# psc0628/NeRF-PRV

Hardware: AMD Instinct MI355X
Metric: ray-samples/s (field evaluations composited; candidate views rendered + scored; scene baseline, field 256^3) (higher is better)
Workload: dtype f16

## Files before the change

### nerf_prv_amd/csrc/prv_api.cpp

```cpp
#include <hip/hip_runtime.h>

#include <algorithm>
#include <atomic>
#include <chrono>
#include <cmath>
#include <cstdarg>
#include <cstdio>
#include <cstdlib>
#include <cstring>
#include <memory>
#include <new>
#include <stdexcept>
#include <string>
#include <vector>

#include "prv_json.hpp"
#include "prv_kernels.hpp"
#include "prv_mesh.hpp"
#include "prv_levels.hpp"
#include "prv_ingp.hpp"
#include "prv_train.hpp"

using namespace prv;

// ... 29 lines not shown
  CamDev* dev = nullptr;
  int device = 0;
  int width = 0, height = 0;
  bool dataset = false;
};

static void train_detach_all(struct prv_ctx* c);
static void comm_detach_all(struct prv_ctx* c);
static void mesh_detach_all(struct prv_ctx* c);

struct prv_ctx {
  int device = 0;
  int n_cu = 256;
  hipStream_t own_stream = nullptr;
  hipStream_t stream = nullptr;
  std::vector<hipStream_t> idle_queues;
  hipStream_t capture_stream = nullptr;
  std::vector<Buffer> idle_buffers;
  size_t idle_bytes = 0;
  std::string err;
  Model models[PRV_MAX_SLOTS];
  Buffer queue, queue_ext, stage, counters, view_ids, img_f32, partial, records, dbg[6];
  Buffer stage_depth;
  Buffer counters_multi, occ_multi;
  int march_multi = -1;
  Buffer img_u8[PRV_MAX_MODELS];
  bool profiling = false;
  std::vector<hipEvent_t> ev_render, ev_march;
  std::vector<hipEvent_t> ev_free;
  std::vector<float> last_render_ms;
  void* pin = nullptr;
  size_t pin_cap = 0;
  hipEvent_t pin_ev = nullptr;
  int blocks_per_cu = -1;
  int cell_cache = -1;
  std::vector<struct prv_trainer*> trainers;
  std::vector<struct prv_comm*> comms;
  std::vector<struct prv_mesh*> meshes;
  float mesh_ms[4] = {0, 0, 0, 0};
  int queue_segments = 8;
  int spatial_regions = 1;
  int pool_on = -1;
  int merge_max = -1;
  size_t stage_budget = (size_t)4 << 30;
  size_t queue_budget = (size_t)8 << 30;
  double coverage_weight = PRV_COVERAGE_WEIGHT_DEFAULT;
// ... 490 lines not shown
  }
  if (!c->pin_ev) HIPCHK(c, hipEventCreateWithFlags(&c->pin_ev, hipEventDisableTiming));
  else HIPCHK(c, hipEventSynchronize(c->pin_ev));
  CamDev* cams = (CamDev*)c->pin;
  int* ids = (int*)((char*)c->pin + (size_t)n_views * sizeof(CamDev));
  int rc;
  if ((rc = gather_cams(c, cs, view_ids, n_views, W, H, cams)) != PRV_OK) return rc;
  for (int i = 0; i < n_views; i++) {
    set_cull_rect(cams[i], box, W, H);
    ids[i] = i;
  }
  if ((rc = ensure(c, c->view_ids, up_bytes)) != PRV_OK) return rc;
  HIPCHK(c, hipMemcpyAsync(c->view_ids.p, c->pin, up_bytes, hipMemcpyHostToDevice, c->stream));
  HIPCHK(c, hipEventRecord(c->pin_ev, c->stream));
  up.cams = cams;
  up.cams_dev = (const CamDev*)c->view_ids.p;
  up.ids_dev = (const int*)((char*)c->view_ids.p + (size_t)n_views * sizeof(CamDev));
  return PRV_OK;
}

constexpr int kSubRegions = 8, kMaxSegments = 8 * kSubRegions;
constexpr size_t kStatOffset = (size_t)kMaxSegments * 128;
constexpr size_t kCountersBytes = kStatOffset + 72 * 8;

struct MarchLayout {
  int spp, n_sub, n_seg;
  int spp_inner_log2 = 0, tile_w_log2, tile_h_log2;
  uint32_t tiles_x, tiles_y;
  MarchLayout(const prv_ctx* c, int W, int H, int spp_) : spp(spp_) {
    n_sub = c->spatial_regions ? kSubRegions : 1;
    n_seg = c->queue_segments * n_sub;
    if (spp > 1 && spp <= 64 && (spp & (spp - 1)) == 0)
      while ((1 << spp_inner_log2) < spp) spp_inner_log2++;
    const int pix_log2 = 8 - spp_inner_log2;
    tile_w_log2 = (pix_log2 + 1) / 2;
    tile_h_log2 = pix_log2 / 2;
    tiles_x = (uint32_t)((W + (1 << tile_w_log2) - 1) >> tile_w_log2);
    tiles_y = (uint32_t)((H + (1 << tile_h_log2) - 1) >> tile_h_log2);
  }
  size_t blocks(size_t n_views) const { return (size_t)tiles_x * tiles_y * n_views * (size_t)(spp_inner_log2 > 0 ? 1 : spp); }
  size_t seg_cap(size_t n_views) const { return ((blocks(n_views) + n_seg - 1) / n_seg) * 256 + 64; }
};

template <class PT>
void march_common(PT& mp, const prv_ctx* c, const MarchLayout& L, const prv_render_opts* o, const Upload& up, size_t v0,
                  size_t n_views, unsigned long long* stat) {
// ... 59 lines not shown
  rp.queue_count = q.queue_count;
  rp.queue_head = queue_head;
  rp.n_segments = L.n_seg;
  rp.n_sub = L.n_sub;
  rp.seg_cap = seg_cap;
  rp.stat_evaluated = stat;
  rp.out_f32 = q.out_f32;
  rp.out_u8 = q.out_u8;
  rp.min_T = o->min_transmittance;
  rp.last_pass = o->spp == 1;
  memcpy(rp.bg, o->background, sizeof(rp.bg));
  render_policy(c, m, (size_t)o->width * o->height, o->step_mode == PRV_STEP_NGP, rp);
  return rp;
}

int render_views(prv_ctx* c, int slot, const prv_camset* cs, const int* view_ids, int n_views,
                 const prv_render_opts* o, float* out_f32, uint8_t* out_u8, bool zero_stats, bool private_output = false,
                 float* out_depth = nullptr, float* out_entropy = nullptr, float* out_alpha = nullptr) {
  if (o->spp != 1 || out_u8 || out_depth) private_output = false;
  const Model& m = c->models[slot];
  const int W = o->width, H = o->height, spp = o->spp;
  const size_t npix = (size_t)W * H;
  int rc;
  if ((rc = ensure(c, c->counters, kCountersBytes)) != PRV_OK) return rc;
  uint32_t* q_head = (uint32_t*)c->counters.p;
  uint32_t* q_count = (uint32_t*)c->counters.p + kMaxSegments * 16;
  unsigned long long* stat = (unsigned long long*)((char*)c->counters.p + kStatOffset);
  if (n_views == 0) {
    if (zero_stats) HIPCHK(c, hipMemsetAsync(stat, 0, kCountersBytes - kStatOffset, c->stream));
    return PRV_OK;
  }
  Upload up;
  if ((rc = upload_views(c, cs, view_ids, n_views, W, H, box_of(m), up)) != PRV_OK) return rc;

  const bool ngp = o->step_mode == PRV_STEP_NGP;
  const size_t slot_bytes = kRecordBytes + (ngp ? kExtBytes : 0);
  size_t batch = std::max<size_t>(1, c->queue_budget / (npix * slot_bytes * (size_t)spp));
  batch = std::min<size_t>(batch, (size_t)n_views);
  const size_t stage_px = out_entropy ? 4 + 4 : out_depth ? 16 + 4 : 16;
  if (spp > 1) batch = std::min<size_t>(batch, std::max<size_t>(1, c->stage_budget / (npix * stage_px * (size_t)spp)));
  if (batch * npix * (size_t)spp >= (1ull << 32)) batch = ((1ull << 32) - 1) / (npix * (size_t)spp);
  if (batch == 0) return fail(c, PRV_E_INVALID, "image x spp too large");
  const MarchLayout L(c, W, H, spp);
  const size_t seg_cap_max = L.seg_cap(batch);
  if (seg_cap_max * (size_t)L.n_seg >= (1ull << 32)) return fail(c, PRV_E_INVALID, "image x spp too large");
  if ((rc = ensure(c, c->queue, seg_cap_max * (size_t)L.n_seg * kRecordBytes)) != PRV_OK) return rc;
  if (ngp && (rc = ensure(c, c->queue_ext, seg_cap_max * (size_t)L.n_seg * kExtBytes)) != PRV_OK) return rc;
  if (spp > 1 && (rc = ensure(c, c->stage, batch * npix * (size_t)spp * (out_entropy ? 4 : 16))) != PRV_OK) return rc;
  if (spp > 1 && (out_depth || out_entropy) && (rc = ensure(c, c->stage_depth, batch * npix * (size_t)spp * 4)) != PRV_OK) return rc;

  const int n_blocks = render_blocks(c, m, npix);
  for (size_t b0 = 0; b0 < (size_t)n_views; b0 += batch) {
    const int nb = (int)std::min(batch, (size_t)n_views - b0);
    float* dst_f32 = out_f32 ? out_f32 + b0 * npix * 4 : nullptr;
    uint32_t* dst_u8 = out_u8 ? (uint32_t*)out_u8 + b0 * npix : nullptr;
    float* dst_depth = out_depth ? out_depth + b0 * npix : nullptr;
    float* depth_target = spp > 1 ? (float*)c->stage_depth.p : dst_depth;
    if (out_depth) HIPCHK(c, hipMemsetAsync(depth_target, 0, (size_t)nb * npix * (size_t)spp * 4, c->stream));
    float* dst_entropy = out_entropy ? out_entropy + b0 * npix : nullptr;
    float* dst_alpha = out_entropy ? out_alpha + b0 * npix : nullptr;
    float* entropy_target = spp > 1 ? (float*)c->stage_depth.p : dst_entropy;
    float* alpha_target = spp > 1 ? (float*)c->stage.p : dst_alpha;
    if (out_entropy) {
      HIPCHK(c, hipMemsetAsync(entropy_target, 0, (size_t)nb * npix * (size_t)spp * 4, c->stream));
      HIPCHK(c, hipMemsetAsync(alpha_target, 0, (size_t)nb * npix * (size_t)spp * 4, c->stream));
    }
    HIPCHK(c, hipMemsetAsync(c->counters.p, 0, b0 == 0 && zero_stats ? kCountersBytes : kStatOffset, c->stream));
    MarchParams mp;
    march_common(mp, c, L, o, up, b0, (size_t)nb, stat);
    mp.field = m.dev;
    mp.S = o->samples_per_ray;
    mp.step_mode = o->step_mode;
    mp.queue = c->queue.p;
    mp.queue_ext = (uint4*)c->queue_ext.p;
    mp.queue_count = q_count;
    mp.out_f32 = out_entropy ? nullptr : spp > 1 ? (float*)c->stage.p : dst_f32;
    mp.out_u8 = spp > 1 ? nullptr : dst_u8;
    if (private_output) {
      const uint64_t tw = 1ull << mp.tile_w_log2, th = 1ull << mp.tile_h_log2;
      uint64_t live_max = 0;
      for (int i = 0; i < nb; i++) {
        const CamDev& cv = up.cams[b0 + i];
        uint64_t w = mp.tiles_x, h = mp.tiles_y;
        if (cv.cull[2] > 0) {
          const uint64_t x0 = (uint64_t)cv.cull[0] / tw, y0 = (uint64_t)cv.cull[1] / th;
          const uint64_t x1 = std::min<uint64_t>(mp.tiles_x, ((uint64_t)cv.cull[2] + tw - 1) / tw);
          const uint64_t y1 = std::min<uint64_t>(mp.tiles_y, ((uint64_t)std::max(cv.cull[3], 0) + th - 1) / th);
          w = x1 > x0 ? x1 - x0 : 0;
          h = y1 > y0 ? y1 - y0 : 0;
        }
// ... 40 lines not shown
int render_ensemble_ngp(prv_ctx* c, const int* slots, int E, const prv_camset* cs, const int* view_ids, int n_views,
                        const prv_render_opts* o, float* scratch_f32, uint8_t* const* out_u8, bool* done) {
  *done = false;
  if (o->step_mode != PRV_STEP_NGP || !march_multi_supported(E) || n_views == 0) return PRV_OK;
  if (c->march_multi == 0) return PRV_OK;
  if (c->march_multi < 0 && E < 3) return PRV_OK;
  const Model& m0 = c->models[slots[0]];
  for (int e = 1; e < E; e++) {
    const Model& m = c->models[slots[e]];
    if (m.desc.occ_res != m0.desc.occ_res || (m.dev.occ_coarse == nullptr) != (m0.dev.occ_coarse == nullptr)) return PRV_OK;
    for (int f = 0; f < e; f++)
      if (slots[f] == slots[e]) return PRV_OK;
  }
  const int W = o->width, H = o->height, spp = o->spp;
  const size_t npix = (size_t)W * H;
  const size_t slot_bytes = kRecordBytes + kExtBytes;
  if ((size_t)n_views * npix * (size_t)spp >= (1ull << 32)) return PRV_OK;
  if ((size_t)n_views * npix * (size_t)spp * slot_bytes > c->queue_budget) return PRV_OK;
  if (spp > 1 && (size_t)n_views * npix * (size_t)spp * 16 > c->stage_budget) return PRV_OK;
  const MarchLayout L(c, W, H, spp);
  const size_t seg_cap = L.seg_cap((size_t)n_views);
  if (seg_cap * (size_t)L.n_seg >= (1ull << 32)) return PRV_OK;
  int rc;
  if ((rc = ensure(c, c->counters, kCountersBytes)) != PRV_OK) return rc;
  if ((rc = ensure(c, c->counters_multi, (size_t)E * kStatOffset)) != PRV_OK) return rc;
  unsigned long long* stat = (unsigned long long*)((char*)c->counters.p + kStatOffset);
  const size_t R = (size_t)m0.desc.occ_res, n_fine = R * R * R, Rc = R / 4, n_coarse = Rc * Rc * Rc;
  if ((rc = ensure(c, c->occ_multi, n_fine + n_coarse + 64)) != PRV_OK) return rc;
  const size_t q_stride = seg_cap * (size_t)L.n_seg * kRecordBytes, x_stride = seg_cap * (size_t)L.n_seg * kExtBytes,
               s_stride = spp > 1 ? (size_t)n_views * npix * (size_t)spp * 16 : 0;
  {
    const size_t grow = (q_stride * (size_t)E > c->queue.bytes ? q_stride * (size_t)E - c->queue.bytes : 0) +
                        (x_stride * (size_t)E > c->queue_ext.bytes ? x_stride * (size_t)E - c->queue_ext.bytes : 0) +
                        (s_stride * (size_t)E > c->stage.bytes ? s_stride * (size_t)E - c->stage.bytes : 0);
    size_t free_b = 0, total_b = 0;
    if (grow && (hipMemGetInfo(&free_b, &total_b) != hipSuccess || grow + ((size_t)2 << 30) > free_b + c->idle_bytes)) return PRV_OK;
  }

  const OccBox box = union_box(c, slots, E);
  Upload up;
  if ((rc = upload_views(c, cs, view_ids, n_views, W, H, box, up)) != PRV_OK) return rc;

  const bool have_coarse = m0.dev.occ_coarse != nullptr;
  {
    OccInterleaveParams ip{};
    ip.n_members = E;
    for (int e = 0; e < E; e++) ip.bits[e] = c->models[slots[e]].dev.occ;
    ip.n_cells = (uint32_t)n_fine;
    ip.out = (uint8_t*)c->occ_multi.p;
    HIPCHK(c, launch_occ_interleave(ip, c->stream));
    if (have_coarse) {
      for (int e = 0; e < E; e++) ip.bits[e] = c->models[slots[e]].dev.occ_coarse;
      ip.n_cells = (uint32_t)n_coarse;
      ip.out = (uint8_t*)c->occ_multi.p + n_fine;
      HIPCHK(c, launch_occ_interleave(ip, c->stream));
    }
  }

  if ((rc = ensure(c, c->queue, q_stride * (size_t)E)) != PRV_OK) return rc;
  if ((rc = ensure(c, c->queue_ext, x_stride * (size_t)E)) != PRV_OK) return rc;
  if (spp > 1 && (rc = ensure(c, c->stage, s_stride * (size_t)E)) != PRV_OK) return rc;
  HIPCHK(c, hipMemsetAsync(c->counters.p, 0, kCountersBytes, c->stream));
  HIPCHK(c, hipMemsetAsync(c->counters_multi.p, 0, (size_t)E * kStatOffset, c->stream));

  MarchMultiParams mp;
  march_common(mp, c, L, o, up, 0, (size_t)n_views, stat);
  mp.occ_bytes = (const uint8_t*)c->occ_multi.p;
  mp.occ_coarse_bytes = have_coarse ? (const uint8_t*)c->occ_multi.p + n_fine : nullptr;
  mp.occ_res = (int)R;
  for (int a = 0; a < 3; a++) {
    mp.occ_lo[a] = box.occ_lo[a];
    mp.occ_hi[a] = box.occ_hi[a];
  }
  mp.n_members = E;
  for (int e = 0; e < E; e++) {
    MarchMember& mm = mp.mem[e];
    mm.queue = (char*)c->queue.p + q_stride * (size_t)e;
    mm.queue_ext = (uint4*)((char*)c->queue_ext.p + x_stride * (size_t)e);
    mm.queue_count = (uint32_t*)((char*)c->counters_multi.p + (size_t)e * kStatOffset) + kMaxSegments * 16;
    mm.out_f32 = spp > 1 ? (float*)((char*)c->stage.p + s_stride * (size_t)e) : scratch_f32;
    mm.out_u8 = spp > 1 ? nullptr : (uint32_t*)out_u8[e];
  }
  if ((rc = timed(c, c->ev_march, [&] { HIPCHK(c, launch_march_multi(mp, n_views, spp, c->stream)); return PRV_OK; })) != PRV_OK) return rc;

  for (int e = 0; e < E; e++) {
    const Model& m = c->models[slots[e]];
    const int n_blocks = render_blocks(c, m, npix);
    uint32_t* q_head = (uint32_t*)((char*)c->counters_multi.p + (size_t)e * kStatOffset);
    const RenderParams rp = render_params(c, m, o, L, mp.seg_cap, mp.mem[e], q_head, stat);
    if ((rc = timed(c, c->ev_render, [&] { HIPCHK(c, launch_render(rp, n_blocks, c->stream)); return PRV_OK; })) != PRV_OK) return rc;
    if (spp > 1)
      HIPCHK(c, launch_spp_reduce((const float*)mp.mem[e].out_f32, (size_t)n_views * npix, spp, o->background, scratch_f32, (uint32_t*)out_u8[e], c->stream));
  }
  *done = true;
  return PRV_OK;
}

int fetch_stats(prv_ctx* c, const prv_render_opts* o, int n_views, int n_models, prv_stats* st) {
  if (!st) return PRV_OK;
  unsigned long long ev[72] = {0};
  HIPCHK(c, hipMemcpyAsync(ev, (char*)c->counters.p + kStatOffset, sizeof(ev), hipMemcpyDeviceToHost, c->stream));
  HIPCHK(c, hipStreamSynchronize(c->stream));
  st->wave_rounds = ev[1];
  st->rays = (uint64_t)n_views * n_models * o->width * o->height * o->spp;
  st->samples_nominal = st->rays * (uint64_t)(o->step_mode == PRV_STEP_NGP ? kNgpMaxSteps : o->samples_per_ray);
  st->samples_evaluated = ev[0];
  st->samples_live = 0;
  for (int s = 0; s < 8; s++) st->samples_live += ev[8 * (1 + s)];
  return PRV_OK;
}

int score_blocks(size_t npix) { return (int)std::min<size_t>(64, std::max<size_t>(1, (npix + 4095) / 4096)); }

}


extern "C" {

int prv_abi_version(void) { return PRV_ABI_VERSION; }

int prv_device_count(void) {
  int n = 0;
  if (hipGetDeviceCount(&n) != hipSuccess) return 0;
  return n;
// ... 670 lines not shown
} catch (...) { return caught(c); }


static int score_ensemble_dev(prv_ctx* c, int method, const uint8_t* const* imgs, int E, int n_views, size_t npix,
                              prv_score_record* rec_dev) {
  const size_t per_view = npix * (method == PRV_SCORE_ENSEMBLE_RGB ? 3 : 2) * sizeof(double);
  const int batch = (int)std::min<size_t>((size_t)n_views, std::max<size_t>(1, ((size_t)1 << 30) / per_view));
  const int nblk = (int)std::min<size_t>(1024, std::max<size_t>(1, (npix + 255) / 256));
  int rc;
  if ((rc = ensure(c, c->partial, (size_t)batch * per_view)) != PRV_OK) return rc;
  EnsembleParams P;
  memset(&P, 0, sizeof(P));
  for (int e = 0; e < E; e++) P.imgs[e] = (const uint32_t*)imgs[e];
  P.E = E;
  P.pixels_per_view = npix;
  P.partial = (double*)c->partial.p;
  for (int v0 = 0; v0 < n_views; v0 += batch) {
    P.view0 = v0;
    HIPCHK(c, launch_score_ensemble(P, method, std::min(batch, n_views - v0), nblk, rec_dev, c->stream));
  }
  return PRV_OK;
}

static int score_psnr_dev(prv_ctx* c, const float* rgba, const float* gt, int n_views, size_t npix, const float bg[4],
                          double coverage_weight, prv_score_record* rec_dev, const CamDev* cams_dev = nullptr, int W = 0) {
  const int nblk = score_blocks(npix);
  int rc;
  if ((rc = ensure(c, c->partial, (size_t)n_views * nblk * 3 * sizeof(double))) != PRV_OK) return rc;
  PsnrParams P;
  memset(&P, 0, sizeof(P));
  P.rgba = rgba;
  P.gt = gt;
  P.pixels_per_view = npix;
  P.cams = cams_dev;
  P.W = W;
  memcpy(P.bg, bg, sizeof(P.bg));
  P.partial = (double*)c->partial.p;
  HIPCHK(c, launch_score_psnr(P, n_views, nblk, c->stream));
  HIPCHK(c, launch_score_finalize(P.partial, n_views, nblk, PRV_SCORE_PSNR_COVERAGE, npix, coverage_weight, rec_dev, c->stream));
  return PRV_OK;
}

int prv_score_ensemble_images(prv_ctx* c, int method, const uint8_t* const* imgs, int E, int n_views, size_t npix,
                              prv_score_record* rec_host) try {
  if (!c) return PRV_E_INVALID;
  if (method != PRV_SCORE_ENSEMBLE_RGB && method != PRV_SCORE_ENSEMBLE_RGB_DENSITY)
    return fail(c, PRV_E_INVALID, "method %d is not an ensemble score", method);
  if (!imgs || E < 1 || E > PRV_MAX_MODELS || n_views < 0 || !rec_host) return fail(c, PRV_E_INVALID, "bad argument");
  if (n_views == 0) return PRV_OK;
  if (npix == 0) return fail(c, PRV_E_INVALID, "empty images");
  HIPCHK(c, hipSetDevice(c->device));
  int rc;
  for (int e = 0; e < E; e++)
    if (!imgs[e]) return fail(c, PRV_E_INVALID, "image set %d is NULL", e);
    else if ((rc = check_device_ptr(c, imgs[e], "rgba8_dev")) != PRV_OK) return rc;
  if ((rc = ensure(c, c->records, (size_t)n_views * sizeof(prv_score_record))) != PRV_OK) return rc;
  if ((rc = score_ensemble_dev(c, method, imgs, E, n_views, npix, (prv_score_record*)c->records.p)) != PRV_OK) return rc;
  return prv_memcpy_d2h(c, rec_host, c->records.p, (size_t)n_views * sizeof(prv_score_record));
} catch (...) { return caught(c); }

int prv_score_psnr_images(prv_ctx* c, const float* rgba, const float* gt, int n_views, size_t npix, const float bg[4],
// ... 63 lines not shown
  return PRV_OK;
} catch (...) { return caught(c); }

int prv_score_views(prv_ctx* c, int method, const int* model_slots, int n_models, const prv_camset* cs,
                    const int* view_ids, int n_views, const prv_render_opts* o, const float* gt,
                    prv_score_record* rec_host, prv_score_record* rec_dev, prv_stats* st) try {
  if (!c) return PRV_E_INVALID;
  int rc;
  if ((rc = check_opts(c, o)) != PRV_OK) return rc;
  if (!cs || !model_slots || n_views < 0) return fail(c, PRV_E_INVALID, "bad argument");
  const bool ens = method == PRV_SCORE_ENSEMBLE_RGB || method == PRV_SCORE_ENSEMBLE_RGB_DENSITY;
  const bool entropy = method == PRV_SCORE_RAY_ENTROPY;
  if (!ens && !entropy && method != PRV_SCORE_PSNR_COVERAGE) return fail(c, PRV_E_INVALID, "unknown score method %d", method);
  if (ens && (n_models < 1 || n_models > PRV_MAX_MODELS)) return fail(c, PRV_E_INVALID, "ensemble size %d", n_models);
  if (entropy && (n_models != 1 || gt)) return fail(c, PRV_E_INVALID, "method 7 scores one model and takes no reference images");
  if (!ens && !entropy && (n_models != 1 || !gt)) return fail(c, PRV_E_INVALID, "method 5 needs one model and reference images");
  for (int e = 0; e < n_models; e++)
    if ((rc = check_model(c, model_slots[e])) != PRV_OK) return rc;
  HIPCHK(c, hipSetDevice(c->device));
  if ((rc = check_device_ptr(c, gt, "gt_rgba_dev")) != PRV_OK || (rc = check_device_ptr(c, rec_dev, "records_dev")) != PRV_OK) return rc;
  const size_t npix = (size_t)o->width * o->height;
  if ((rc = ensure(c, c->records, std::max<size_t>(16, (size_t)n_views * sizeof(prv_score_record)))) != PRV_OK) return rc;
  prv_score_record* rec = (prv_score_record*)c->records.p;
  if ((rc = ensure(c, c->img_f32, std::max<size_t>(16, (size_t)n_views * npix * (entropy ? 8 : 16)))) != PRV_OK) return rc;
  if (entropy) {
    float* hp = (float*)c->img_f32.p;
    float* ap = hp + (size_t)n_views * npix;
    if ((rc = render_views(c, model_slots[0], cs, view_ids, n_views, o, nullptr, nullptr, true, o->spp == 1, nullptr, hp, ap)) != PRV_OK) return rc;
    if (n_views) {
      const int nblk = score_blocks(npix);
      if ((rc = ensure(c, c->partial, (size_t)n_views * nblk * 2 * sizeof(double))) != PRV_OK) return rc;
      HIPCHK(c, launch_score_entropy(hp, ap, npix, n_views, nblk, (double*)c->partial.p, c->stream));
      HIPCHK(c, launch_score_finalize((const double*)c->partial.p, n_views, nblk, PRV_SCORE_RAY_ENTROPY, npix, 0.0, rec, c->stream));
    }
  } else if (ens) {
    const uint8_t* imgs[PRV_MAX_MODELS];
    uint8_t* out8[PRV_MAX_MODELS];
    for (int e = 0; e < n_models; e++) {
      if ((rc = ensure(c, c->img_u8[e], std::max<size_t>(16, (size_t)n_views * npix * 4))) != PRV_OK) return rc;
      imgs[e] = (const uint8_t*)c->img_u8[e].p;
      out8[e] = (uint8_t*)c->img_u8[e].p;
    }
    bool one_march = false;
    if ((rc = render_ensemble_ngp(c, model_slots, n_models, cs, view_ids, n_views, o, (float*)c->img_f32.p, out8, &one_march)) != PRV_OK) return rc;
    for (int e = 0; e < n_models && !one_march; e++)
      if ((rc = render_views(c, model_slots[e], cs, view_ids, n_views, o, (float*)c->img_f32.p, out8[e], e == 0)) != PRV_OK) return rc;
    if (n_views && (rc = score_ensemble_dev(c, method, imgs, n_models, n_views, npix, rec)) != PRV_OK) return rc;
  } else {
    const bool priv = o->spp == 1;
    if ((rc = render_views(c, model_slots[0], cs, view_ids, n_views, o, (float*)c->img_f32.p, nullptr, true, priv)) != PRV_OK)
      return rc;
    if (n_views && (rc = score_psnr_dev(c, (const float*)c->img_f32.p, gt, n_views, npix, o->background, c->coverage_weight, rec,
                                        priv ? (const CamDev*)c->view_ids.p : nullptr, o->width)) != PRV_OK)
      return rc;
  }
  if (rec_dev && n_views)
    HIPCHK(c, hipMemcpyAsync(rec_dev, rec, (size_t)n_views * sizeof(prv_score_record), hipMemcpyDeviceToDevice, c->stream));
  if (rec_host && n_views) {
    HIPCHK(c, hipMemcpyAsync(rec_host, rec, (size_t)n_views * sizeof(prv_score_record), hipMemcpyDeviceToHost, c->stream));
    HIPCHK(c, hipStreamSynchronize(c->stream));
  }
  return fetch_stats(c, o, n_views, n_models, st);
} catch (...) { return caught(c); }

int prv_argmax(const prv_score_record* r, const int* ids, int n) {
  if (!r || !ids) return -1;
  double best = -1e100;
  int best_id = -1;
  for (int i = 0; i < n; i++)
    if (r[i].score > best) {
      best = r[i].score;
      best_id = ids[i];
    }
  return best_id;
}

int prv_rank(const prv_score_record* r, const int* ids, int n, int* order) try {
  if (n < 0 || (n > 0 && (!r || !ids || !order))) return PRV_E_INVALID;
  std::vector<int> idx(n);
  for (int i = 0; i < n; i++) idx[i] = i;
  std::stable_sort(idx.begin(), idx.end(), [&](int a, int b) {
    const bool na = std::isnan(r[a].score), nb = std::isnan(r[b].score);
    if (na != nb) return nb;
    if (!na && r[a].score != r[b].score) return r[a].score > r[b].score;
    return ids[a] < ids[b];
  });
  for (int i = 0; i < n; i++) order[i] = ids[idx[i]];
  return PRV_OK;
} catch (...) { return caught(nullptr); }


int prv_debug_render_clock(prv_ctx* c, uint64_t* shader_cycles, uint64_t* ref_ticks, double* ref_hz) try {
  if (!c) return PRV_E_INVALID;
  HIPCHK(c, hipSetDevice(c->device));
  if (!shader_cycles || !ref_ticks || !ref_hz) return fail(c, PRV_E_INVALID, "NULL output");
  if (!c->counters.p) return fail(c, PRV_E_STATE, "nothing rendered yet");
  unsigned long long v[2] = {0, 0};
  HIPCHK(c, hipMemcpyAsync(v, (char*)c->counters.p + kStatOffset + 16, 16, hipMemcpyDeviceToHost, c->stream));
  HIPCHK(c, hipStreamSynchronize(c->stream));
  int khz = 0;
  HIPCHK(c, hipDeviceGetAttribute(&khz, hipDeviceAttributeWallClockRate, c->device));
  *shader_cycles = v[0];
  *ref_ticks = v[1];
  *ref_hz = (double)khz * 1e3;
  return PRV_OK;
} catch (...) { return caught(c); }

int prv_debug_model_layout(prv_ctx* c, int slot, prv_model_layout* out) try {
  if (!c) return PRV_E_INVALID;
  int rc = check_model(c, slot);
  if (rc != PRV_OK) return rc;
  if (!out) return fail(c, PRV_E_INVALID, "out is NULL");
  const Model& m = c->models[slot];
  HostLevel lv[kMaxLevels];
  uint64_t total = 0;
  compute_levels(m.desc, lv, &total);
  out->table_bytes_canonical = m.table_halfs * 2;
  out->table_bytes_physical = m.phys_bytes;
  out->kernel_features = m.dev.n_features;
  out->kernel_dense_levels = render_instance_dense_levels(m.dev);
  out->kernel_slots = 64;
  out->n_dense_levels = m.dev.n_dense_levels;
  out->n_hashed_levels = 0;
  for (int l = 0; l < m.desc.n_levels; l++) out->n_hashed_levels += lv[l].hashed ? 1 : 0;
  return PRV_OK;
} catch (...) { return caught(c); }

int prv_debug_raygen(prv_ctx* c, const prv_camset* cs, int view, int W, int H, int spp_k, float* o, float* d, float* t) try {
  if (!c) return PRV_E_INVALID;
// ... 58 lines not shown
```

### nerf_prv_amd/csrc/prv_kernels.hip

```cpp
#include "prv_kernels.hpp"

#include <algorithm>

#ifndef PRV_ABLATE
#define PRV_ABLATE 0
#endif

namespace prv {


__device__ __forceinline__ void morton16(uint32_t i, uint32_t& x, uint32_t& y) {
  x = (i & 1u) | ((i >> 1) & 2u) | ((i >> 2) & 4u) | ((i >> 3) & 8u);
  y = ((i >> 1) & 1u) | ((i >> 2) & 2u) | ((i >> 3) & 4u) | ((i >> 4) & 8u);
}

constexpr float kNgpDt = 1.7320508075688772f / 1024.0f;

__device__ __forceinline__ uint32_t march_ngp(const FieldDev& fd, const float o[3], const float d[3], float t0, float t1,
                                              uint32_t (*mw)[256], int& k_lo, int& k_hi, int& first_nz, int& last_nz) {
  const float dt = kNgpDt;
  first_nz = 32;
  last_nz = -1;
  k_lo = k_hi = 0;
  float ta = t0, tb = t1;
// ... 1130 lines not shown
    double* b = buf[c & 1];
#pragma unroll
    for (int j = 0; j < 8; j++) b[j * 64 + lane] = r[j];
    __syncthreads();
    if (c + 1 < n_chunks) {
#pragma unroll
      for (int j = 0; j < 8; j++) {
        const size_t i = (c + 1) * 512 + (size_t)j * 64 + lane;
        r[j] = i < n_terms ? t[i] : 0.0;
      }
    }
#pragma unroll 16
    for (int i = 0; i < 512; i++) sum += b[i];
  }
  if (lane == 0) {
    prv_score_record out;
    out.score = sum;
    out.psnr = 0.f;
    out.coverage = 0.f;
    rec[v] = out;
  }
}

__global__ __launch_bounds__(256) void score_psnr_kernel(PsnrParams P) {
  __shared__ double sm[4];
  const int v = blockIdx.y;
  const size_t npix = P.pixels_per_view;
  const float4* img = reinterpret_cast<const float4*>(P.rgba) + (size_t)v * npix;
  const float4* gt = reinterpret_cast<const float4*>(P.gt) + (size_t)v * npix;
  double se = 0.0, cov = 0.0, unc = 0.0;
  int c0 = 0, c1 = 0, c2 = 0, c3 = 0;
  if (P.cams && P.cams[v].cull[2] > 0) {
    c0 = P.cams[v].cull[0]; c1 = P.cams[v].cull[1]; c2 = P.cams[v].cull[2]; c3 = P.cams[v].cull[3];
  }
  for (size_t p = (size_t)blockIdx.x * 256 + threadIdx.x; p < npix; p += (size_t)gridDim.x * 256) {
    float4 a4 = make_float4(0.f, 0.f, 0.f, 0.f);
    bool inside = true;
    if (c2 > 0) {
      const int y = (int)((uint32_t)p / (uint32_t)P.W), x = (int)((uint32_t)p - (uint32_t)y * (uint32_t)P.W);
      inside = x >= c0 && x < c2 && y >= c1 && y < c3;
    }
    if (inside) a4 = img[p];
    const float4 r4 = gt[p];
    const float ra = 1.0f - a4.w, rg = 1.0f - r4.w;
    const float av[3] = {a4.x, a4.y, a4.z}, rv[3] = {r4.x, r4.y, r4.z};
#pragma unroll
    for (int k = 0; k < 3; k++) {
      float a = fmaf(ra, P.bg[k], av[k]);
      float rr = fmaf(rg, P.bg[k], rv[k]);
      a = fminf(fmaxf(linear_to_srgb(a), 0.0f), 1.0f);
      rr = fminf(fmaxf(linear_to_srgb(rr), 0.0f), 1.0f);
      double dlt = (double)a - (double)rr;
      se += dlt * dlt;
    }
    cov += (double)a4.w;
    const double u = 1.0 - (double)a4.w;
    unc += u * u;
  }
  double s0 = block_reduce_sum(se, sm);
  double s1 = block_reduce_sum(cov, sm);
  double s2 = block_reduce_sum(unc, sm);
  if (threadIdx.x == 0) {
    P.partial[((size_t)v * gridDim.x + blockIdx.x) * 3 + 0] = s0;
    P.partial[((size_t)v * gridDim.x + blockIdx.x) * 3 + 1] = s1;
    P.partial[((size_t)v * gridDim.x + blockIdx.x) * 3 + 2] = s2;
  }
}

__global__ __launch_bounds__(256) void score_entropy_kernel(const float* __restrict__ entropy, const float* __restrict__ alpha,
                                                            size_t npix, double* __restrict__ partial) {
  __shared__ double sm[4];
  const int v = blockIdx.y;
  const float* hv = entropy + (size_t)v * npix;
  const float* av = alpha + (size_t)v * npix;
  double sh = 0.0, sa = 0.0;
  for (size_t p = (size_t)blockIdx.x * 256 + threadIdx.x; p < npix; p += (size_t)gridDim.x * 256) {
    sh += (double)hv[p];
    sa += (double)av[p];
  }
  const double s0 = block_reduce_sum(sh, sm);
// ... 62 lines not shown
#pragma unroll
      for (int i = 0; i < 5; i++) s = fmaf(tap[i], r[i][k], s);
      q[k] = s;
    }
    const float mA = q[0], mB = q[1];
    const float sA = q[2] - mA * mA, sB = q[3] - mB * mB, sAB = q[4] - mA * mB;
    const float p1 = (2.0f * mA * mB + c1) / (mA * mA + mB * mB + c1);
    const float p2 = (2.0f * sAB + c2) / (sA + sB + c2);
    acc += (double)(p1 * p2);
  }
  const double s = block_reduce_sum(acc, sm);
  if (threadIdx.x == 0) partial[(size_t)v * gridDim.x + blockIdx.x] = s;
}

__global__ void ssim_finalize_kernel(const double* __restrict__ partial, int n_views, int n_blocks, double count,
                                     double* __restrict__ out) {
  const int v = blockIdx.x * blockDim.x + threadIdx.x;
  if (v >= n_views) return;
  double s = 0.0;
  for (int b = 0; b < n_blocks; b++) s += partial[(size_t)v * n_blocks + b];
  out[v] = s / count;
}

__global__ void score_finalize_kernel(const double* __restrict__ partial, int n_views, int n_blocks,
                                      int method, size_t pixels_per_view, double coverage_weight,
                                      prv_score_record* __restrict__ rec) {
  const int v = blockIdx.x * blockDim.x + threadIdx.x;
  if (v >= n_views) return;
  prv_score_record out;
  out.psnr = 0.f;
  out.coverage = 0.f;
  if (method == PRV_SCORE_PSNR_COVERAGE) {
    double se = 0.0, cov = 0.0, unc = 0.0;
    for (int b = 0; b < n_blocks; b++) {
      se += partial[((size_t)v * n_blocks + b) * 3 + 0];
      cov += partial[((size_t)v * n_blocks + b) * 3 + 1];
      unc += partial[((size_t)v * n_blocks + b) * 3 + 2];
    }
    const double mse = se / (double)(pixels_per_view * 3);
    const double psnr = -10.0 * log10(mse);
    out.score = -psnr + coverage_weight * (unc / (double)pixels_per_view);
    out.psnr = (float)psnr;
    out.coverage = (float)(cov / (double)pixels_per_view);
  } else if (method == PRV_SCORE_RAY_ENTROPY) {
    double sh = 0.0, sa = 0.0;
    for (int b = 0; b < n_blocks; b++) {
      sh += partial[((size_t)v * n_blocks + b) * 2 + 0];
      sa += partial[((size_t)v * n_blocks + b) * 2 + 1];
    }
    out.score = sh / (double)pixels_per_view;
    out.coverage = (float)(sa / (double)pixels_per_view);
  } else {
    double s = 0.0;
    for (int b = 0; b < n_blocks; b++) s += partial[(size_t)v * n_blocks + b];
    out.score = s;
  }
  rec[v] = out;
}


__device__ __forceinline__ unsigned long long mix64(unsigned long long z) {
  z = (z ^ (z >> 30)) * 0xBF58476D1CE4E5B9ull;
  z = (z ^ (z >> 27)) * 0x94D049BB133111EBull;
  return z ^ (z >> 31);
}

__global__ __launch_bounds__(256) void synth_table_kernel(uint16_t* __restrict__ table, size_t n,
                                                          unsigned long long seed, float amp) {
  for (size_t i = (size_t)blockIdx.x * 256 + threadIdx.x; i < n; i += (size_t)gridDim.x * 256) {
    unsigned long long hsh = mix64(seed + 1ull * 0xD1B54A32D192ED03ull + (unsigned long long)i * 0x9E3779B97F4A7C15ull);
    uint32_t u = (uint32_t)(hsh >> 40);
    float v = (float)u * (1.0f / 8388608.0f) - 1.0f;
    _Float16 hv = to_half(v * amp);
    table[i] = __builtin_bit_cast(uint16_t, hv);
  }
}

template <int F>
__global__ __launch_bounds__(256) void repack_level_kernel(const uint16_t* __restrict__ canon,
                                                           uint16_t* __restrict__ phys, RepackLevel L) {
// ... 332 lines not shown
                     rec + P.view0);
  return hipGetLastError();
}

hipError_t launch_score_psnr(const PsnrParams& P, int n_views, int n_blocks, hipStream_t s) {
  dim3 grid((unsigned)n_blocks, (unsigned)n_views);
  hipLaunchKernelGGL(score_psnr_kernel, grid, dim3(256), 0, s, P);
  return hipGetLastError();
}

hipError_t launch_ssim(const float* img, const float* gt, int n_views, int W, int H, const float bg[4], float* la,
                       float* lb, double* partial, int n_blocks, double* out, hipStream_t s) {
  const size_t n = (size_t)n_views * W * H;
  unsigned blocks = (unsigned)std::min<size_t>(4096, (n + 255) / 256);
  hipLaunchKernelGGL(ssim_lum_kernel, dim3(blocks), dim3(256), 0, s, reinterpret_cast<const float4*>(img),
                     reinterpret_cast<const float4*>(gt), n, bg[0], bg[1], bg[2], bg[3], la, lb);
  hipLaunchKernelGGL(ssim_map_kernel, dim3((unsigned)n_blocks, (unsigned)n_views), dim3(256), 0, s, la, lb, W, H, partial);
  hipLaunchKernelGGL(ssim_finalize_kernel, dim3((unsigned)((n_views + 63) / 64)), dim3(64), 0, s, partial, n_views,
                     n_blocks, (double)(W - 4) * (double)(H - 4), out);
  return hipGetLastError();
}

hipError_t launch_score_finalize(const double* partial, int n_views, int n_blocks, int method,
                                 size_t pixels_per_view, double coverage_weight, prv_score_record* rec, hipStream_t s) {
  hipLaunchKernelGGL(score_finalize_kernel, dim3((unsigned)((n_views + 63) / 64)), dim3(64), 0, s, partial,
                     n_views, n_blocks, method, pixels_per_view, coverage_weight, rec);
  return hipGetLastError();
}

hipError_t launch_synth_table(uint16_t* table, size_t n, uint64_t seed, float amp, hipStream_t s) {
  hipLaunchKernelGGL(synth_table_kernel, dim3(2048), dim3(256), 0, s, table, n, (unsigned long long)seed, amp);
  return hipGetLastError();
}

hipError_t launch_repack_level(const uint16_t* canon, uint16_t* phys, const RepackLevel& L, int F, hipStream_t s) {
  unsigned blocks = ((L.hashed ? L.n : L.res * L.res * L.res) + 255) / 256;
  if (blocks > 8192) blocks = 8192;
  if (blocks == 0) return hipSuccess;
  if (F == 4)
    hipLaunchKernelGGL(repack_level_kernel<4>, dim3(blocks), dim3(256), 0, s, canon, phys, L);
  else
    hipLaunchKernelGGL(repack_level_kernel<2>, dim3(blocks), dim3(256), 0, s, canon, phys, L);
  return hipGetLastError();
}

hipError_t launch_debug_raygen(const CamDev& cam, int W, int H, int spp_k, float* o, float* d, float* t,
                               hipStream_t s) {
  hipLaunchKernelGGL(debug_raygen_kernel, dim3((unsigned)((W * H + 255) / 256)), dim3(256), 0, s, cam, W, H,
                     spp_k, o, d, t);
// ... 21 lines not shown
```

### nerf_prv_amd/csrc/prv_kernels.hpp

```cpp
#pragma once
#include "../../include/prv.h"
#include "prv_device.hpp"

namespace prv {

constexpr size_t kRecordBytes = 96;
constexpr int kRecordWords = 6;
constexpr uint32_t kClaim = 64;
constexpr int kMaxSamples = 128;
constexpr int kNgpMaxSteps = PRV_NGP_MAX_STEPS;
constexpr int kExtChunks = kNgpMaxSteps / 128 - 1;
constexpr size_t kExtBytes = (size_t)kExtChunks * 16;

struct MarchParams {
  FieldDev field;
  const CamDev* cams;
  const int* view_ids;
  int W, H, S;
  uint32_t tiles_x, tiles_y;
  int tile_w_log2, tile_h_log2;
  int spp_inner_log2;
  int live_grid;
  uint32_t live_tiles_max;
  int step_mode;
// ... 113 lines not shown
hipError_t launch_render_depth(const RenderDepthParams& P, int n_blocks, hipStream_t s);
hipError_t launch_spp_reduce_depth(const float* stage, size_t n_pixels, int spp, float* out, hipStream_t s);
hipError_t launch_render_entropy(const RenderEntropyParams& P, int n_blocks, hipStream_t s);
hipError_t launch_score_entropy(const float* entropy, const float* alpha, size_t npix, int n_views, int n_blocks, double* partial,
                                hipStream_t s);
int render_instance_dense_levels(const FieldDev& fd);
struct PreceptPose {
  double w2c[16], c2w[16];
};
hipError_t launch_precept(const FieldDev& fd, const float* voxels, int n, const PreceptPose& pose, const Rs2Intr& in,
                          float max_range, int32_t* out, hipStream_t s);
hipError_t launch_first_hit(const FieldDev& fd, const CamDev* cams, int n_views, int W, int H, float max_range,
                            int32_t* out, hipStream_t s);
hipError_t launch_splat_points(const float* xyz, const uint8_t* rgb, size_t n, float scale, const float off[3],
                               const CamDev* cams, int n_views, int W, int H, int point_size, int flip180,
                               unsigned long long* zbuf, uint32_t* out, hipStream_t s);
hipError_t launch_quantize(const float* in, size_t n, const float bg[4], uint8_t* out, hipStream_t s);
hipError_t launch_score_ensemble(const EnsembleParams& P, int method, int n_views, int n_blocks, prv_score_record* rec,
                                 hipStream_t s);
hipError_t launch_score_psnr(const PsnrParams& P, int n_views, int n_blocks, hipStream_t s);
hipError_t launch_ssim(const float* img, const float* gt, int n_views, int W, int H, const float bg[4], float* la,
                       float* lb, double* partial, int n_blocks, double* out, hipStream_t s);
hipError_t launch_score_finalize(const double* partial, int n_views, int n_blocks, int method,
                                 size_t pixels_per_view, double coverage_weight, prv_score_record* rec, hipStream_t s);
hipError_t launch_synth_table(uint16_t* table, size_t n, uint64_t seed, float amp, hipStream_t s);
hipError_t launch_debug_raygen(const CamDev& cam, int W, int H, int spp_k, float* o, float* d, float* t,
                               hipStream_t s);
hipError_t launch_debug_field(const FieldDev& fd, const float* pos, const float* dir, int n, uint16_t* feat,
                              float* out36, int32_t* occ, hipStream_t s);

}
```

Before: 23.97 billion.

## Double-buffer counters cleared by finalize kernel, unroll PSNR scoring and parallelize finalize

Splits the counters buffer into two halves. The score finalize kernel zeroes the idle half, so the next render round can skip its counter memset. The finalize kernel now writes the secondary record output directly, which removes a device-to-device copy, and it sums block partials with one wavefront per view using shuffles instead of a serial loop per thread. The PSNR kernel is unrolled with nontemporal ground-truth loads and incremental pixel coordinates. The cost is more state tracking of which half is clean, with a risk of stale counters if the sequence of calls differs from what is expected.

Measured after the change: 24.06 billion (median of 6 runs). Within noise of the previous version (+0.3%).

```diff
diff --git a/nerf_prv_amd/csrc/prv_api.cpp b/nerf_prv_amd/csrc/prv_api.cpp
--- a/nerf_prv_amd/csrc/prv_api.cpp
+++ b/nerf_prv_amd/csrc/prv_api.cpp
@@ -75,6 +75,8 @@
   Model models[PRV_MAX_SLOTS];
   Buffer queue, queue_ext, stage, counters, view_ids, img_f32, partial, records, dbg[6];
   Buffer stage_depth;
+  int ctr_cur = 0, ctr_clean = -1;
+  uint64_t n_memsets = 0;
   Buffer counters_multi, occ_multi;
   int march_multi = -1;
   Buffer img_u8[PRV_MAX_MODELS];
@@ -611,6 +613,18 @@
 constexpr int kSubRegions = 8, kMaxSegments = 8 * kSubRegions;
 constexpr size_t kStatOffset = (size_t)kMaxSegments * 128;
 constexpr size_t kCountersBytes = kStatOffset + 72 * 8;
+constexpr size_t kCountersStride = (kCountersBytes + 255) & ~(size_t)255;
+static_assert(kCountersBytes % 16 == 0, "score_finalize_kernel clears a half in 16-byte words");
+
+int ensure_counters(prv_ctx* c) {
+  if (!c->counters.p || c->counters.bytes < 2 * kCountersStride) c->ctr_clean = -1;
+  return ensure(c, c->counters, 2 * kCountersStride);
+}
+char* counters_half(const prv_ctx* c, int half) { return (char*)c->counters.p + (size_t)half * kCountersStride; }
+hipError_t stream_fill(prv_ctx* c, void* p, size_t bytes) {
+  c->n_memsets++;
+  return hipMemsetAsync(p, 0, bytes, c->stream);
+}
 
 struct MarchLayout {
   int spp, n_sub, n_seg;
@@ -716,12 +730,18 @@
   const int W = o->width, H = o->height, spp = o->spp;
   const size_t npix = (size_t)W * H;
   int rc;
-  if ((rc = ensure(c, c->counters, kCountersBytes)) != PRV_OK) return rc;
-  uint32_t* q_head = (uint32_t*)c->counters.p;
-  uint32_t* q_count = (uint32_t*)c->counters.p + kMaxSegments * 16;
-  unsigned long long* stat = (unsigned long long*)((char*)c->counters.p + kStatOffset);
+  if ((rc = ensure_counters(c)) != PRV_OK) return rc;
+  const bool pre_cleared = zero_stats && n_views > 0 && c->ctr_clean == (c->ctr_cur ^ 1);
+  if (pre_cleared) {
+    c->ctr_cur ^= 1;
+    c->ctr_clean = -1;
+  }
+  char* ctr = counters_half(c, c->ctr_cur);
+  uint32_t* q_head = (uint32_t*)ctr;
+  uint32_t* q_count = (uint32_t*)ctr + kMaxSegments * 16;
+  unsigned long long* stat = (unsigned long long*)(ctr + kStatOffset);
   if (n_views == 0) {
-    if (zero_stats) HIPCHK(c, hipMemsetAsync(stat, 0, kCountersBytes - kStatOffset, c->stream));
+    if (zero_stats) HIPCHK(c, stream_fill(c, stat, kCountersBytes - kStatOffset));
     return PRV_OK;
   }
   Upload up;
@@ -750,16 +770,16 @@
     uint32_t* dst_u8 = out_u8 ? (uint32_t*)out_u8 + b0 * npix : nullptr;
     float* dst_depth = out_depth ? out_depth + b0 * npix : nullptr;
     float* depth_target = spp > 1 ? (float*)c->stage_depth.p : dst_depth;
-    if (out_depth) HIPCHK(c, hipMemsetAsync(depth_target, 0, (size_t)nb * npix * (size_t)spp * 4, c->stream));
+    if (out_depth) HIPCHK(c, stream_fill(c, depth_target, (size_t)nb * npix * (size_t)spp * 4));
     float* dst_entropy = out_entropy ? out_entropy + b0 * npix : nullptr;
     float* dst_alpha = out_entropy ? out_alpha + b0 * npix : nullptr;
     float* entropy_target = spp > 1 ? (float*)c->stage_depth.p : dst_entropy;
     float* alpha_target = spp > 1 ? (float*)c->stage.p : dst_alpha;
     if (out_entropy) {
-      HIPCHK(c, hipMemsetAsync(entropy_target, 0, (size_t)nb * npix * (size_t)spp * 4, c->stream));
-      HIPCHK(c, hipMemsetAsync(alpha_target, 0, (size_t)nb * npix * (size_t)spp * 4, c->stream));
-    }
-    HIPCHK(c, hipMemsetAsync(c->counters.p, 0, b0 == 0 && zero_stats ? kCountersBytes : kStatOffset, c->stream));
+      HIPCHK(c, stream_fill(c, entropy_target, (size_t)nb * npix * (size_t)spp * 4));
+      HIPCHK(c, stream_fill(c, alpha_target, (size_t)nb * npix * (size_t)spp * 4));
+    }
+    if (!(b0 == 0 && pre_cleared)) HIPCHK(c, stream_fill(c, ctr, b0 == 0 && zero_stats ? kCountersBytes : kStatOffset));
     MarchParams mp;
     march_common(mp, c, L, o, up, b0, (size_t)nb, stat);
     mp.field = m.dev;
@@ -846,9 +866,9 @@
   const size_t seg_cap = L.seg_cap((size_t)n_views);
   if (seg_cap * (size_t)L.n_seg >= (1ull << 32)) return PRV_OK;
   int rc;
-  if ((rc = ensure(c, c->counters, kCountersBytes)) != PRV_OK) return rc;
+  if ((rc = ensure_counters(c)) != PRV_OK) return rc;
   if ((rc = ensure(c, c->counters_multi, (size_t)E * kStatOffset)) != PRV_OK) return rc;
-  unsigned long long* stat = (unsigned long long*)((char*)c->counters.p + kStatOffset);
+  unsigned long long* stat = (unsigned long long*)(counters_half(c, c->ctr_cur) + kStatOffset);
   const size_t R = (size_t)m0.desc.occ_res, n_fine = R * R * R, Rc = R / 4, n_coarse = Rc * Rc * Rc;
   if ((rc = ensure(c, c->occ_multi, n_fine + n_coarse + 64)) != PRV_OK) return rc;
   const size_t q_stride = seg_cap * (size_t)L.n_seg * kRecordBytes, x_stride = seg_cap * (size_t)L.n_seg * kExtBytes,
@@ -884,8 +904,8 @@
   if ((rc = ensure(c, c->queue, q_stride * (size_t)E)) != PRV_OK) return rc;
   if ((rc = ensure(c, c->queue_ext, x_stride * (size_t)E)) != PRV_OK) return rc;
   if (spp > 1 && (rc = ensure(c, c->stage, s_stride * (size_t)E)) != PRV_OK) return rc;
-  HIPCHK(c, hipMemsetAsync(c->counters.p, 0, kCountersBytes, c->stream));
-  HIPCHK(c, hipMemsetAsync(c->counters_multi.p, 0, (size_t)E * kStatOffset, c->stream));
+  HIPCHK(c, stream_fill(c, counters_half(c, c->ctr_cur), kCountersBytes));
+  HIPCHK(c, stream_fill(c, c->counters_multi.p, (size_t)E * kStatOffset));
 
   MarchMultiParams mp;
   march_common(mp, c, L, o, up, 0, (size_t)n_views, stat);
@@ -923,7 +943,7 @@
 int fetch_stats(prv_ctx* c, const prv_render_opts* o, int n_views, int n_models, prv_stats* st) {
   if (!st) return PRV_OK;
   unsigned long long ev[72] = {0};
-  HIPCHK(c, hipMemcpyAsync(ev, (char*)c->counters.p + kStatOffset, sizeof(ev), hipMemcpyDeviceToHost, c->stream));
+  HIPCHK(c, hipMemcpyAsync(ev, counters_half(c, c->ctr_cur) + kStatOffset, sizeof(ev), hipMemcpyDeviceToHost, c->stream));
   HIPCHK(c, hipStreamSynchronize(c->stream));
   st->wave_rounds = ev[1];
   st->rays = (uint64_t)n_views * n_models * o->width * o->height * o->spp;
@@ -1640,8 +1660,18 @@
   return PRV_OK;
 }
 
+static int finalize_round(prv_ctx* c, int n_views, int nblk, int method, size_t npix, double coverage_weight, prv_score_record* rec,
+                          prv_score_record* rec2) {
+  const int other = c->ctr_cur ^ 1;
+  HIPCHK(c, launch_score_finalize((const double*)c->partial.p, n_views, nblk, method, npix, coverage_weight, rec, c->stream, rec2,
+                                  counters_half(c, other), kCountersBytes));
+  c->ctr_clean = other;
+  return PRV_OK;
+}
+
 static int score_psnr_dev(prv_ctx* c, const float* rgba, const float* gt, int n_views, size_t npix, const float bg[4],
-                          double coverage_weight, prv_score_record* rec_dev, const CamDev* cams_dev = nullptr, int W = 0) {
+                          double coverage_weight, prv_score_record* rec_dev, const CamDev* cams_dev = nullptr, int W = 0,
+                          bool round = false, prv_score_record* rec2 = nullptr) {
   const int nblk = score_blocks(npix);
   int rc;
   if ((rc = ensure(c, c->partial, (size_t)n_views * nblk * 3 * sizeof(double))) != PRV_OK) return rc;
@@ -1655,6 +1685,7 @@
   memcpy(P.bg, bg, sizeof(P.bg));
   P.partial = (double*)c->partial.p;
   HIPCHK(c, launch_score_psnr(P, n_views, nblk, c->stream));
+  if (round) return finalize_round(c, n_views, nblk, PRV_SCORE_PSNR_COVERAGE, npix, coverage_weight, rec_dev, rec2);
   HIPCHK(c, launch_score_finalize(P.partial, n_views, nblk, PRV_SCORE_PSNR_COVERAGE, npix, coverage_weight, rec_dev, c->stream));
   return PRV_OK;
 }
@@ -1764,6 +1795,7 @@
   const size_t npix = (size_t)o->width * o->height;
   if ((rc = ensure(c, c->records, std::max<size_t>(16, (size_t)n_views * sizeof(prv_score_record)))) != PRV_OK) return rc;
   prv_score_record* rec = (prv_score_record*)c->records.p;
+  bool rec_dev_written = false;
   if ((rc = ensure(c, c->img_f32, std::max<size_t>(16, (size_t)n_views * npix * (entropy ? 8 : 16)))) != PRV_OK) return rc;
   if (entropy) {
     float* hp = (float*)c->img_f32.p;
@@ -1773,7 +1805,8 @@
       const int nblk = score_blocks(npix);
       if ((rc = ensure(c, c->partial, (size_t)n_views * nblk * 2 * sizeof(double))) != PRV_OK) return rc;
       HIPCHK(c, launch_score_entropy(hp, ap, npix, n_views, nblk, (double*)c->partial.p, c->stream));
-      HIPCHK(c, launch_score_finalize((const double*)c->partial.p, n_views, nblk, PRV_SCORE_RAY_ENTROPY, npix, 0.0, rec, c->stream));
+      if ((rc = finalize_round(c, n_views, nblk, PRV_SCORE_RAY_ENTROPY, npix, 0.0, rec, rec_dev)) != PRV_OK) return rc;
+      rec_dev_written = true;
     }
   } else if (ens) {
     const uint8_t* imgs[PRV_MAX_MODELS];
@@ -1793,10 +1826,11 @@
     if ((rc = render_views(c, model_slots[0], cs, view_ids, n_views, o, (float*)c->img_f32.p, nullptr, true, priv)) != PRV_OK)
       return rc;
     if (n_views && (rc = score_psnr_dev(c, (const float*)c->img_f32.p, gt, n_views, npix, o->background, c->coverage_weight, rec,
-                                        priv ? (const CamDev*)c->view_ids.p : nullptr, o->width)) != PRV_OK)
+                                        priv ? (const CamDev*)c->view_ids.p : nullptr, o->width, true, rec_dev)) != PRV_OK)
       return rc;
-  }
-  if (rec_dev && n_views)
+    rec_dev_written = n_views > 0;
+  }
+  if (rec_dev && n_views && !rec_dev_written)
     HIPCHK(c, hipMemcpyAsync(rec_dev, rec, (size_t)n_views * sizeof(prv_score_record), hipMemcpyDeviceToDevice, c->stream));
   if (rec_host && n_views) {
     HIPCHK(c, hipMemcpyAsync(rec_host, rec, (size_t)n_views * sizeof(prv_score_record), hipMemcpyDeviceToHost, c->stream));
@@ -1838,7 +1872,7 @@
   if (!shader_cycles || !ref_ticks || !ref_hz) return fail(c, PRV_E_INVALID, "NULL output");
   if (!c->counters.p) return fail(c, PRV_E_STATE, "nothing rendered yet");
   unsigned long long v[2] = {0, 0};
-  HIPCHK(c, hipMemcpyAsync(v, (char*)c->counters.p + kStatOffset + 16, 16, hipMemcpyDeviceToHost, c->stream));
+  HIPCHK(c, hipMemcpyAsync(v, counters_half(c, c->ctr_cur) + kStatOffset + 16, 16, hipMemcpyDeviceToHost, c->stream));
   HIPCHK(c, hipStreamSynchronize(c->stream));
   int khz = 0;
   HIPCHK(c, hipDeviceGetAttribute(&khz, hipDeviceAttributeWallClockRate, c->device));
@@ -1847,6 +1881,12 @@
   *ref_hz = (double)khz * 1e3;
   return PRV_OK;
 } catch (...) { return caught(c); }
+
+int prv_debug_stream_memsets(prv_ctx* c, uint64_t* n) {
+  if (!c || !n) return PRV_E_INVALID;
+  *n = c->n_memsets;
+  return PRV_OK;
+}
 
 int prv_debug_model_layout(prv_ctx* c, int slot, prv_model_layout* out) try {
   if (!c) return PRV_E_INVALID;
diff --git a/nerf_prv_amd/csrc/prv_kernels.hip b/nerf_prv_amd/csrc/prv_kernels.hip
--- a/nerf_prv_amd/csrc/prv_kernels.hip
+++ b/nerf_prv_amd/csrc/prv_kernels.hip
@@ -1176,40 +1176,67 @@
   }
 }
 
+__device__ __forceinline__ void psnr_add_pixel(const float4 a4, const float4 r4, const float bg[4], double& se, double& cov, double& unc) {
+  const float ra = 1.0f - a4.w, rg = 1.0f - r4.w;
+  const float av[3] = {a4.x, a4.y, a4.z}, rv[3] = {r4.x, r4.y, r4.z};
+#pragma unroll
+  for (int k = 0; k < 3; k++) {
+    float a = fmaf(ra, bg[k], av[k]);
+    float rr = fmaf(rg, bg[k], rv[k]);
+    a = fminf(fmaxf(linear_to_srgb(a), 0.0f), 1.0f);
+    rr = fminf(fmaxf(linear_to_srgb(rr), 0.0f), 1.0f);
+    double dlt = (double)a - (double)rr;
+    se += dlt * dlt;
+  }
+  cov += (double)a4.w;
+  const double u = 1.0 - (double)a4.w;
+  unc += u * u;
+}
+
+constexpr int kPsnrUnroll = 4;
 __global__ __launch_bounds__(256) void score_psnr_kernel(PsnrParams P) {
+  typedef float f4v __attribute__((ext_vector_type(4)));
   __shared__ double sm[4];
   const int v = blockIdx.y;
   const size_t npix = P.pixels_per_view;
   const float4* img = reinterpret_cast<const float4*>(P.rgba) + (size_t)v * npix;
-  const float4* gt = reinterpret_cast<const float4*>(P.gt) + (size_t)v * npix;
+  const f4v* gt = reinterpret_cast<const f4v*>(P.gt) + (size_t)v * npix;
   double se = 0.0, cov = 0.0, unc = 0.0;
   int c0 = 0, c1 = 0, c2 = 0, c3 = 0;
   if (P.cams && P.cams[v].cull[2] > 0) {
     c0 = P.cams[v].cull[0]; c1 = P.cams[v].cull[1]; c2 = P.cams[v].cull[2]; c3 = P.cams[v].cull[3];
   }
-  for (size_t p = (size_t)blockIdx.x * 256 + threadIdx.x; p < npix; p += (size_t)gridDim.x * 256) {
-    float4 a4 = make_float4(0.f, 0.f, 0.f, 0.f);
-    bool inside = true;
-    if (c2 > 0) {
-      const int y = (int)((uint32_t)p / (uint32_t)P.W), x = (int)((uint32_t)p - (uint32_t)y * (uint32_t)P.W);
-      inside = x >= c0 && x < c2 && y >= c1 && y < c3;
-    }
-    if (inside) a4 = img[p];
-    const float4 r4 = gt[p];
-    const float ra = 1.0f - a4.w, rg = 1.0f - r4.w;
-    const float av[3] = {a4.x, a4.y, a4.z}, rv[3] = {r4.x, r4.y, r4.z};
-#pragma unroll
-    for (int k = 0; k < 3; k++) {
-      float a = fmaf(ra, P.bg[k], av[k]);
-      float rr = fmaf(rg, P.bg[k], rv[k]);
-      a = fminf(fmaxf(linear_to_srgb(a), 0.0f), 1.0f);
-      rr = fminf(fmaxf(linear_to_srgb(rr), 0.0f), 1.0f);
-      double dlt = (double)a - (double)rr;
-      se += dlt * dlt;
-    }
-    cov += (double)a4.w;
-    const double u = 1.0 - (double)a4.w;
-    unc += u * u;
+  const size_t p0 = (size_t)blockIdx.x * 256 + threadIdx.x, stride = (size_t)gridDim.x * 256;
+  const size_t n = p0 < npix ? (npix - p0 + stride - 1) / stride : 0;
+  uint32_t x = 0, y = 0, dx = 0, dy = 0;
+  if (c2 > 0) {
+    y = (uint32_t)p0 / (uint32_t)P.W;
+    x = (uint32_t)p0 - y * (uint32_t)P.W;
+    dy = (uint32_t)stride / (uint32_t)P.W;
+    dx = (uint32_t)stride - dy * (uint32_t)P.W;
+  }
+  size_t p = p0;
+  for (size_t k = 0; k < n; k += kPsnrUnroll) {
+    float4 a4[kPsnrUnroll], r4[kPsnrUnroll];
+#pragma unroll
+    for (int u = 0; u < kPsnrUnroll; u++) {
+      a4[u] = r4[u] = make_float4(0.f, 0.f, 0.f, 0.f);
+      if (k + u < n) {
+        const f4v g = __builtin_nontemporal_load(gt + p);
+        r4[u] = make_float4(g.x, g.y, g.z, g.w);
+        if (c2 <= 0 || ((int)x >= c0 && (int)x < c2 && (int)y >= c1 && (int)y < c3)) a4[u] = img[p];
+      }
+      p += stride;
+      x += dx;
+      y += dy;
+      if (x >= (uint32_t)P.W && c2 > 0) {
+        x -= (uint32_t)P.W;
+        y++;
+      }
+    }
+#pragma unroll
+    for (int u = 0; u < kPsnrUnroll; u++)
+      if (k + u < n) psnr_add_pixel(a4[u], r4[u], P.bg, se, cov, unc);
   }
   double s0 = block_reduce_sum(se, sm);
   double s1 = block_reduce_sum(cov, sm);
@@ -1318,40 +1345,54 @@
   out[v] = s / count;
 }
 
-__global__ void score_finalize_kernel(const double* __restrict__ partial, int n_views, int n_blocks,
-                                      int method, size_t pixels_per_view, double coverage_weight,
-                                      prv_score_record* __restrict__ rec) {
-  const int v = blockIdx.x * blockDim.x + threadIdx.x;
-  if (v >= n_views) return;
+template <int K>
+__device__ __forceinline__ void sum_block_partials(const double* __restrict__ partial, int v, int n_blocks, double (&s)[K]) {
+  const int lane = threadIdx.x & 63;
+#pragma unroll
+  for (int k = 0; k < K; k++) s[k] = 0.0;
+  for (int b0 = 0; b0 < n_blocks; b0 += 64) {
+    double mine[K];
+#pragma unroll
+    for (int k = 0; k < K; k++) mine[k] = b0 + lane < n_blocks ? partial[((size_t)v * n_blocks + b0 + lane) * K + k] : 0.0;
+    const int nb = min(64, n_blocks - b0);
+    for (int j = 0; j < nb; j++) {
+#pragma unroll
+      for (int k = 0; k < K; k++) s[k] += __shfl(mine[k], j);
+    }
+  }
+}
+
+__global__ __launch_bounds__(64) void score_finalize_kernel(const double* __restrict__ partial, int n_views, int n_blocks,
+                                                            int method, size_t pixels_per_view, double coverage_weight,
+                                                            prv_score_record* __restrict__ rec, prv_score_record* __restrict__ rec2,
+                                                            uint4* __restrict__ clear, uint32_t clear_n) {
+  const int v = blockIdx.x;
+  for (uint32_t i = blockIdx.x * 64u + threadIdx.x; i < clear_n; i += gridDim.x * 64u) clear[i] = make_uint4(0u, 0u, 0u, 0u);
   prv_score_record out;
   out.psnr = 0.f;
   out.coverage = 0.f;
   if (method == PRV_SCORE_PSNR_COVERAGE) {
-    double se = 0.0, cov = 0.0, unc = 0.0;
-    for (int b = 0; b < n_blocks; b++) {
-      se += partial[((size_t)v * n_blocks + b) * 3 + 0];
-      cov += partial[((size_t)v * n_blocks + b) * 3 + 1];
-      unc += partial[((size_t)v * n_blocks + b) * 3 + 2];
-    }
-    const double mse = se / (double)(pixels_per_view * 3);
+    double s[3];
+    sum_block_partials<3>(partial, v, n_blocks, s);
+    const double mse = s[0] / (double)(pixels_per_view * 3);
     const double psnr = -10.0 * log10(mse);
-    out.score = -psnr + coverage_weight * (unc / (double)pixels_per_view);
+    out.score = -psnr + coverage_weight * (s[2] / (double)pixels_per_view);
     out.psnr = (float)psnr;
-    out.coverage = (float)(cov / (double)pixels_per_view);
+    out.coverage = (float)(s[1] / (double)pixels_per_view);
   } else if (method == PRV_SCORE_RAY_ENTROPY) {
-    double sh = 0.0, sa = 0.0;
-    for (int b = 0; b < n_blocks; b++) {
-      sh += partial[((size_t)v * n_blocks + b) * 2 + 0];
-      sa += partial[((size_t)v * n_blocks + b) * 2 + 1];
-    }
-    out.score = sh / (double)pixels_per_view;
-    out.coverage = (float)(sa / (double)pixels_per_view);
+    double s[2];
+    sum_block_partials<2>(partial, v, n_blocks, s);
+    out.score = s[0] / (double)pixels_per_view;
+    out.coverage = (float)(s[1] / (double)pixels_per_view);
   } else {
-    double s = 0.0;
-    for (int b = 0; b < n_blocks; b++) s += partial[(size_t)v * n_blocks + b];
-    out.score = s;
-  }
-  rec[v] = out;
+    double s[1];
+    sum_block_partials<1>(partial, v, n_blocks, s);
+    out.score = s[0];
+  }
+  if (threadIdx.x == 0) {
+    rec[v] = out;
+    if (rec2) rec2[v] = out;
+  }
 }
 
 
@@ -1730,9 +1771,10 @@
 }
 
 hipError_t launch_score_finalize(const double* partial, int n_views, int n_blocks, int method,
-                                 size_t pixels_per_view, double coverage_weight, prv_score_record* rec, hipStream_t s) {
-  hipLaunchKernelGGL(score_finalize_kernel, dim3((unsigned)((n_views + 63) / 64)), dim3(64), 0, s, partial,
-                     n_views, n_blocks, method, pixels_per_view, coverage_weight, rec);
+                                 size_t pixels_per_view, double coverage_weight, prv_score_record* rec, hipStream_t s,
+                                 prv_score_record* rec2, void* clear, size_t clear_bytes) {
+  hipLaunchKernelGGL(score_finalize_kernel, dim3((unsigned)n_views), dim3(64), 0, s, partial, n_views, n_blocks, method,
+                     pixels_per_view, coverage_weight, rec, rec2, reinterpret_cast<uint4*>(clear), (uint32_t)(clear_bytes / 16));
   return hipGetLastError();
 }
 
diff --git a/nerf_prv_amd/csrc/prv_kernels.hpp b/nerf_prv_amd/csrc/prv_kernels.hpp
--- a/nerf_prv_amd/csrc/prv_kernels.hpp
+++ b/nerf_prv_amd/csrc/prv_kernels.hpp
@@ -159,7 +159,8 @@
 hipError_t launch_ssim(const float* img, const float* gt, int n_views, int W, int H, const float bg[4], float* la,
                        float* lb, double* partial, int n_blocks, double* out, hipStream_t s);
 hipError_t launch_score_finalize(const double* partial, int n_views, int n_blocks, int method,
-                                 size_t pixels_per_view, double coverage_weight, prv_score_record* rec, hipStream_t s);
+                                 size_t pixels_per_view, double coverage_weight, prv_score_record* rec, hipStream_t s,
+                                 prv_score_record* rec2 = nullptr, void* clear = nullptr, size_t clear_bytes = 0);
 hipError_t launch_synth_table(uint16_t* table, size_t n, uint64_t seed, float amp, hipStream_t s);
 hipError_t launch_debug_raygen(const CamDev& cam, int W, int H, int spp_k, float* o, float* d, float* t,
                                hipStream_t s);
```
